# jemisjoky/ContracTN

Hardware: AMD Instinct MI355X
Metric: contractions/sec (MPS-100 overlap, bond=256, phys=4, fp32, stabilised split format) (higher is better)
Workload: dtype f32; 1 GPU; mps_overlap_100sites_D256_d4_zipper_R512; replicas_per_gpu=512, steps_per_contraction=199, bytes_min_per_contraction=205537284, parallelism=replicas x1

## Files before the change

contractn_amd/csrc/engine.hip:

```cpp
#include <hip/hip_runtime.h>

#include <cmath>
#include <cstdio>
#include <cstring>
#include <new>
#include <string>
#include <vector>

#include "plan.h"

#include "kernel_args.h"
#include "kernels_mfma.h"
#include "kernels_mfma_g.h"
#include "kernels_mfma_g64.h"
#include "kernels_mfma_h.h"
#include "kernels_mfma_ares.h"
#include "kernels_zip.h"
#include "kernels_zip64.h"
#include "kernels_zipl.h"
#include "kernels_sweep.h"
#include "kernels_mfma_lat.h"
#include "kernels_stream.h"

namespace ctn {

thread_local std::string g_err;

struct DevSwitches {
  int mfma_g = 1;
  int graph = 1;
  int mfma_bk = 0;
  int group = 1;
  int halve = 1;
  int lat_wg_per_cu_x2 = 2;
  int lat_max_t = 64;
  int splitk_fill_long = 2;
  int lat64_min_k = 512;
  int splitk = -1;
  int splitk_max = 0;
  int lat = -1;
  int hform = -1;
  int sweep = -1;
  int dot_tr = 1;
  int zip = -1;
  int zipl = -1;
  int zipl_max_r = 8;
  int g_big_min_k = 1024;
  int ares = -1;
  int ares_ntw = 0;
  int g_big = 1;
  int g_splitk = 1;
  int zipl_mp = 0;
  bool g_no_asm = false;
  const char* stamps = nullptr;
  int stamp_step = -1;
};
static DevSwitches read_dev_switches() {
  DevSwitches d;
  auto num = [](const char* name, int dflt) { const char* e = getenv(name); return e ? atoi(e) : dflt; };
  d.mfma_g = num("CTN_MFMA_G", 1);
  d.graph = num("CTN_GRAPH", 1);
  const int bk = num("CTN_MFMA_BK", 0);
  d.mfma_bk = (bk == 16 || bk == 32) ? bk : 0;
  d.splitk = num("CTN_SPLITK", -1);
  d.splitk_max = num("CTN_SPLITK_MAX", 0);
  d.lat = num("CTN_LAT", -1);
  d.hform = num("CTN_H", -1);
  d.zip = num("CTN_ZIP", -1);
  d.zipl = num("CTN_ZIPL", -1);
  d.zipl_max_r = num("CTN_ZIPL_MAX_R", 8);
  d.zipl_mp = num("CTN_ZIPL_MP", 0);
  d.g_splitk = num("CTN_G_SPLITK", 1);
  d.g_big = num("CTN_G_BIG", 1);
  d.ares = num("CTN_ARES", -1);
  d.ares_ntw = num("CTN_ARES_NTW", 0);
  d.g_big_min_k = num("CTN_G_BIG_MIN_K", 1024);
  d.dot_tr = num("CTN_DOT_TR", 1);
  d.sweep = num("CTN_SWEEP", -1);
  d.lat64_min_k = num("CTN_LAT64_MIN_K", 512);
  d.splitk_fill_long = num("CTN_SPLITK_FILL_LONG", 2);
  d.lat_max_t = num("CTN_LAT_MAX_T", 64);
  d.lat_wg_per_cu_x2 = num("CTN_LAT_WG_X2", 2);
  d.halve = num("CTN_HALVE_TILES", 1);
  d.group = num("CTN_GROUP", 1);
  d.g_no_asm = getenv("CTN_G_NO_ASM") != nullptr;
  d.stamps = getenv("CTN_DEBUG_STAMPS");
  d.stamp_step = num("CTN_DEBUG_STAMP_STEP", -1);
  return d;
}

#define HIPCHECK(expr)                                                                   \
  do {                                                                                   \
    hipError_t e_ = (expr);                                                              \
    if (e_ != hipSuccess) {                                                              \
      g_err = std::string(#expr) + ": " + hipGetErrorString(e_);                         \
      return CTN_HIP_ERROR;                                                              \
    }                                                                                    \
  } while (0)

struct DeviceGuard {
  int prev = -1;
  hipError_t err;
  explicit DeviceGuard(int dev) {
    if (hipGetDevice(&prev) != hipSuccess) { prev = -1; (void)hipGetLastError(); }
    err = prev == dev ? hipSuccess : hipSetDevice(dev);
    if (prev == dev) prev = -1;
  }
  ~DeviceGuard() { if (prev >= 0) (void)hipSetDevice(prev); }
};

struct Exec {
  const Plan* plan = nullptr;
  int device = 0;
  hipStream_t stream = nullptr;
  bool own_stream = false;
  int R = 1;
  int n_tensors = 0;
  int n_cu = 256;
  DevSwitches sw;
  int mfma_g = 1;
  int use_graph = 1;
  bool graph_warm = false;
  bool graph_aligned = true;
  hipGraphExec_t graph_exec = nullptr;
  struct ZipDesc { bool on = false; int64_t ldE = 0, ldXq = 0, ldXk = 0, ldYq = 0, ldYm = 0, ldC = 0; int Q = 0, U = 0, K1 = 0;
                   int zu = 128; };
  std::vector<ZipDesc> zip;
  std::vector<char> zip_skip;
  struct ZipLat { bool on = false, from_prev = false, feeds_next = false; int buf = 0, mp = 32; ZipDesc d; };
  std::vector<ZipLat> zl;
  std::vector<char> zl_skip;
  float* d_zl_slab[2] = {nullptr, nullptr};
  struct SweepDesc {
    bool on = false;
    std::vector<int> steps;
    int64_t ldIn = 0, ldOut = 0, ldWl = 0, ldWp = 0, ldX = 0;
    int J = 0, M = 0, D = 0, Pd = 0;
  };
  SweepDesc sweep;
  std::vector<char> sweep_role;
  int32_t* d_sweep_ids = nullptr;
  int64_t* d_sweep_off = nullptr;
  int32_t* d_sweep_slots = nullptr;
  double* d_sweep_a = nullptr;
  float* d_sweep_s = nullptr;
  double* d_sweep_z = nullptr;
  double* d_sweep_la = nullptr;
  double* d_sweep_ls = nullptr;
  std::vector<int> ares_ntw;
  struct DotTr { bool on = false; int Ka = 0, Kb = 0, x_is_a = 1; int64_t ldY = 0; };
  std::vector<DotTr> dot_tr;
  std::vector<int32_t> launched_tile;
  char* d_ws = nullptr;
  int32_t* d_tables = nullptr;
  int64_t* d_tables64 = nullptr;
  void** d_ptrs = nullptr;
  std::vector<void*> h_ptrs;
  bool ptrs_valid = false;
  double* d_partials = nullptr;
  double* d_scratch = nullptr;
  void* d_slab = nullptr;
  void* d_slab2 = nullptr;
  std::vector<int> step_partials;
  std::vector<int64_t> step_off;
  int64_t part_slots = 0;
  int64_t* d_stepOff = nullptr;
  int32_t* d_stepSlots = nullptr;
  double* d_log = nullptr;
// ... 617 lines not shown
      z.min_norm = P.min_norm;
      z.partC = E->d_partials + (size_t)E->step_off[s] * R;
      z.partC_stride = E->step_partials[s];
      const bool timed_z = E->timing_runs < E->timing_slots;
      const size_t ez = timed_z ? ((size_t)E->timing_runs * P.n_steps + s) * 2 : 0;
      if (timed_z) HIPCHECK(hipEventRecord(E->events[ez], E->stream));
      if ((int)E->launched_tile.size() != P.n_steps) E->launched_tile.assign(P.n_steps, 0);
      E->launched_tile[s] = (L.mp << 16) | ZM;
      const dim3 gz((unsigned)((int64_t)R * nub * S));
      z.dbg = nullptr;
      if (E->sw.stamps && (E->sw.stamp_step < 0 || E->sw.stamp_step == s)) {
        const size_t need = (size_t)gz.x;
        if (E->dbg_tiles < need) {
          if (E->d_dbg) (void)hipFree(E->d_dbg);
          HIPCHECK(hipMalloc((void**)&E->d_dbg, need * 64));
          E->dbg_tiles = need;
        }
        z.dbg = E->d_dbg;
        HIPCHECK(hipMemsetAsync(E->d_dbg, 0, E->dbg_tiles * 64, E->stream));
      }
      if (zd.Q == 4 && L.mp == 32) hipLaunchKernelGGL((k_zip_lat<4, 32>), gz, dim3(512), 0, E->stream, z);
      else if (zd.Q == 4) hipLaunchKernelGGL((k_zip_lat<4, 64>), gz, dim3(512), 0, E->stream, z);
      else hipLaunchKernelGGL((k_zip_lat<2, 64>), gz, dim3(512), 0, E->stream, z);
      if (!L.feeds_next || eager) {
        hipLaunchKernelGGL(k_zip_slab_sum, dim3((unsigned)E->step_partials[s], (unsigned)R), dim3(256), 0, E->stream,
                           (const float*)z.slabs_out, S, zd.U, (void* const*)E->d_ptrs, E->n_tensors, st.out, zd.ldC, z.partC,
                           z.partC_stride);
        if (eager && P.stabilize && s + 1 < P.n_steps) {
          const int64_t numel = P.tensors[st.out].numel;
          const dim3 g((unsigned)std::max<int64_t>(1, std::min<int64_t>((numel / 4 + 255) / 256, 2048)), R);
          hipLaunchKernelGGL(k_renorm<float>, g, dim3(256), 0, E->stream, (void* const*)E->d_ptrs, E->n_tensors, st.out, numel,
                             (const double*)z.partC, E->step_partials[s], E->step_partials[s], P.min_norm);
        }
      }
      if (timed_z) HIPCHECK(hipEventRecord(E->events[ez + 1], E->stream));
      continue;
    }
    if (!E->zip_skip.empty() && E->zip_skip[s]) {
      if ((int)E->launched_tile.size() != P.n_steps) E->launched_tile.assign(P.n_steps, 0);
      E->launched_tile[s] = (1 << 16) | 1;
      if (E->timing_runs < E->timing_slots) {
        const size_t e0 = ((size_t)E->timing_runs * P.n_steps + s) * 2;
        HIPCHECK(hipEventRecord(E->events[e0], E->stream));
        HIPCHECK(hipEventRecord(E->events[e0 + 1], E->stream));
      }
      continue;
    }
    if (!E->zip.empty() && E->zip[s].on) {
      const Exec::ZipDesc& zd = E->zip[s];
      const Step& s1 = P.steps[s - 1];
      ZipArgs z{};
      z.ptrs = E->d_ptrs; z.n_tensors = E->n_tensors;
      z.idE = s1.lhs; z.idX = s1.rhs; z.idY = st.rhs; z.idC = st.out;
      z.ldE = zd.ldE; z.ldXq = zd.ldXq; z.ldXk = zd.ldXk; z.ldYq = zd.ldYq; z.ldYm = zd.ldYm; z.ldC = zd.ldC;
      z.K1 = zd.K1; z.Q = zd.Q; z.U = zd.U;
      z.partE = nullptr; z.PE = 0; z.strideE = 0; z.numelE = 1.0;
      if (s1.lhs >= P.n_inputs && P.stabilize && !E->eager_rescale && P.steps[P.tensors[s1.lhs].producer].kernel != CTN_KERNEL_FUSED) {
        const int ps = P.tensors[s1.lhs].producer;
        z.partE = E->d_partials + (size_t)E->step_off[ps] * R;
        z.PE = z.strideE = E->step_partials[ps];
        z.numelE = (double)P.tensors[s1.lhs].numel;
      }
      z.min_norm = P.min_norm;
      z.partC = E->d_partials + (size_t)E->step_off[s] * R;
      z.partC_stride = E->step_partials[s];
      z.R = R; z.dbg = nullptr;
      const bool timed_z = E->timing_runs < E->timing_slots;
      const size_t ez = timed_z ? ((size_t)E->timing_runs * P.n_steps + s) * 2 : 0;
      if (timed_z) HIPCHECK(hipEventRecord(E->events[ez], E->stream));
      if ((int)E->launched_tile.size() != P.n_steps) E->launched_tile.assign(P.n_steps, 0);
      E->launched_tile[s] = (512 << 16) | (zd.zu == 64 ? 128 : 256);
      const int per = zd.U / zd.zu;
      if (E->sw.stamps && (E->sw.stamp_step < 0 || E->sw.stamp_step == s)) {
        const size_t need = (size_t)per * R;
        if (E->dbg_tiles < need) {
          if (E->d_dbg) (void)hipFree(E->d_dbg);
          HIPCHECK(hipMalloc((void**)&E->d_dbg, need * 64));
          E->dbg_tiles = need;
        }
        z.dbg = E->d_dbg;
        HIPCHECK(hipMemsetAsync(E->d_dbg, 0, E->dbg_tiles * 64, E->stream));
      }
      if (zd.zu == 64) hipLaunchKernelGGL(k_zip64_f32, dim3((unsigned)((int64_t)per * R)), dim3(512), 0, E->stream, z);
      else hipLaunchKernelGGL(k_zip_f32, dim3((unsigned)((int64_t)per * R)), dim3(512), 0, E->stream, z);
      if (E->eager_rescale && P.stabilize && s + 1 < P.n_steps) {
        const int64_t numel = P.tensors[st.out].numel;
        const dim3 g((unsigned)std::max<int64_t>(1, std::min<int64_t>((numel / 4 + 255) / 256, 2048)), R);
        hipLaunchKernelGGL(k_renorm<float>, g, dim3(256), 0, E->stream, (void* const*)E->d_ptrs, E->n_tensors, st.out, numel,
                           (const double*)z.partC, E->step_partials[s], E->step_partials[s], P.min_norm);
      }
      if (timed_z) HIPCHECK(hipEventRecord(E->events[ez + 1], E->stream));
      continue;
    }
    if (st.kernel == CTN_KERNEL_FUSED) {
      if (E->timing_runs < E->timing_slots) {
        const size_t e0 = ((size_t)E->timing_runs * P.n_steps + s) * 2;
        HIPCHECK(hipEventRecord(E->events[e0], E->stream));
        HIPCHECK(hipEventRecord(E->events[e0 + 1], E->stream));
      }
      continue;
    }
    StepArgs a;
    const int32_t* T = E->d_tables;
    const int64_t* T8 = E->d_tables64;
    a.obA = T8 + st.t.obA; a.obB = T8 + st.t.obB; a.obC = T8 + st.t.obC;
    a.omA = T + st.t.omA; a.omC = T + st.t.omC;
    a.onB = T + st.t.onB; a.onC = T + st.t.onC;
    a.okA = T + st.t.okA; a.okB = T + st.t.okB;
    a.ptrs = E->d_ptrs;
    auto part_of = [&](int id, const double** p, int32_t* cnt, int32_t* stride, double* numel) {
      *p = nullptr; *cnt = 0; *stride = 0; *numel = 1;
      if (id >= P.n_inputs && P.stabilize && !E->eager_rescale && P.steps[P.tensors[id].producer].kernel != CTN_KERNEL_FUSED) {
        const int ps = P.tensors[id].producer;
        *p = E->d_partials + (size_t)E->step_off[ps] * R;
        *cnt = *stride = E->step_partials[ps];
        *numel = (double)P.tensors[id].numel;
      }
    };
    part_of(st.lhs, &a.partA, &a.PA, &a.strideA, &a.numelA);
    part_of(st.rhs, &a.partB, &a.PB, &a.strideB, &a.numelB);
    part_of(st.lhs2, &a.partA2, &a.PA2, &a.strideA2, &a.numelA2);
    a.obA2 = T8 + st.t.obA2; a.omA2 = T + st.t.omA2; a.okA2 = T + st.t.okA2;
    a.idA2 = st.lhs2 >= 0 ? st.lhs2 : E->n_tensors - 1;
    a.krX = st.krX; a.krY = st.krY;
    a.epw = st.epw | (st.epw_split ? 0x100 : 0);
    double* part_dst = E->d_partials + (size_t)E->step_off[s] * R;
    const int part_stride = E->step_partials[s];
    a.partC = st.collapse ? E->d_scratch : part_dst;
    a.partC_stride = st.collapse ? st.blocks : part_stride;
    int collapse_blocks = st.blocks;
    bool reduced = false;
    bool do_collapse = st.collapse;
    a.min_norm = P.min_norm;
    a.Bt = (int32_t)st.Bt; a.M = (int32_t)st.M; a.N = (int32_t)st.N; a.K = (int32_t)st.K;
    a.idA = st.lhs; a.idB = st.rhs >= 0 ? st.rhs : E->n_tensors - 1; a.idC = st.out;
    a.n_tensors = E->n_tensors;
    const int row_tile = (st.kernel == CTN_KERNEL_MFMA_F32 && st.tileM == 64) ? 64 : kTileM;
    a.tiles_m = (int32_t)((st.M + row_tile - 1) / row_tile);
    a.tiles_n = (int32_t)((st.N + kTileN - 1) / kTileN);
    a.blocks_per_replica = st.blocks;
    a.R = R;
    a.c_vec = (st.cvec && (s + 1 < P.n_steps || E->outs_aligned16)) ? 1 : 0;
    a.dbg = nullptr;
    a.ks_slab = nullptr; a.ks_numelC = 0; a.ks_S = 0; a.ks_chunk = 0;
    a.ohA = T8 + st.t.ohA; a.ohB = T8 + st.t.ohB; a.ohC = T8 + st.t.ohC;
    a.olA = T + st.t.olA; a.olB = T + st.t.olB; a.olC = T + st.t.olC;
    a.H = (int32_t)st.H; a.L = (int32_t)st.L; a.Nv = (int32_t)st.Nv;
    a.sAn = (int32_t)st.sAn; a.sBn = (int32_t)st.sBn;
    a.dNq = make_fastdiv((st.Nv + st.vecw - 1) / st.vecw);
    a.dL = make_fastdiv(st.L);
    a.dNv = make_fastdiv(st.Nv);

    const bool timed = E->timing_runs < E->timing_slots;
    const size_t ev0 = timed ? ((size_t)E->timing_runs * P.n_steps + s) * 2 : 0;
    if (timed) HIPCHECK(hipEventRecord(E->events[ev0], E->stream));
    if ((int)E->launched_tile.size() != P.n_steps) E->launched_tile.assign(P.n_steps, 0);
    auto used_tile = [&](int tm, int tn) { E->launched_tile[s] = (tm << 16) | tn; };
    switch (st.kernel) {
      case CTN_KERNEL_MFMA_F32: {
        const int64_t total = (int64_t)st.blocks * R;
        if (total >= (1LL << 31)) { g_err = "grid too large"; return CTN_UNSUPPORTED; }
        if (const int ntw_av = (int)E->ares_ntw.size() == P.n_steps ? E->ares_ntw[s] : 0) {
          const int ntw = ntw_av & 0xffff, avec = ntw_av >> 16;
          const int wgs = (int)(st.Bt * (st.N / AR_TN / ntw));
          a.partC = E->d_scratch; a.partC_stride = wgs;
          do_collapse = true; collapse_blocks = wgs;
          used_tile(256, std::min(AR_TN * ntw, 32768));
// ... 1197 lines not shown
```

contractn_amd/csrc/kernels_zip.h:

```cpp
#pragma once
#include "kernels_mfma_g.h"

namespace ctn {

struct ZipArgs {
  void* const* ptrs;
  int32_t n_tensors, idE, idX, idY, idC;
  int64_t ldE;
  int64_t ldXq, ldXk;
  int64_t ldYq, ldYm;
  int64_t ldC;
  int32_t K1, Q, U;
  const double* partE;
  int32_t PE, strideE;
  double numelE, min_norm;
  double* partC;
  int32_t partC_stride, R;
  unsigned long long* dbg;
};

constexpr int ZM = 256, ZU = 128, ZK = 16, ZSTG = 8192;
constexpr int ZST = 3;

__global__ __launch_bounds__(512, 1) void k_zip_f32(ZipArgs a) {
  __shared__ __attribute__((aligned(16))) float smem[ZST * ZSTG + 16];
  double* red = reinterpret_cast<double*>(smem + ZST * ZSTG);

  const int tid = threadIdx.x;
  const int lane = tid & 63;
  const int w = __builtin_amdgcn_readfirstlane(tid >> 6);
  const int kh = w >> 2, ub = w & 3;
  const int l31 = lane & 31, h = lane >> 5;
  const int nwg = gridDim.x, bid = blockIdx.x;
  const int xcd = bid & 7, slot = bid >> 3, q8 = nwg >> 3, r8 = nwg & 7;
  const int pid = (xcd < r8 ? xcd * (q8 + 1) : r8 * (q8 + 1) + (xcd - r8) * q8) + slot;
  const int per = a.U / ZU;
  const int r = pid / per;
  const int t_ = pid - r * per;
  const int u0 = t_ * ZU;
#ifdef CTN_STAMPS
  if (a.dbg && tid == 0) a.dbg[(size_t)pid * 8 + 0] = __builtin_amdgcn_s_memtime();
#endif
  void* const* tp = a.ptrs + (size_t)r * a.n_tensors;
  const float* __restrict__ E = (const float*)tp[a.idE];
  const float* __restrict__ X = (const float*)tp[a.idX] + u0;
  const float* __restrict__ Y = (const float*)tp[a.idY];
  float* __restrict__ C = (float*)tp[a.idC];

  const int T1 = a.K1 / ZK;
  constexpr int T2 = (ZM / 2) / ZK;
  const int TQ = T1 + T2, TT = a.Q * TQ;

  const float* const rE0 = E + (int64_t)(4 * ub) * a.ldE;
  const float* rE = rE0;
  const float* rX = X + (int64_t)(4 * ub) * a.ldXk;
  const float* rY = Y + (int64_t)(4 * ub) * a.ldYm;
  const int offE = 4 * lane, offX = h * (int)a.ldXk + 4 * l31;
  const int64_t stepE = (int64_t)ZK * a.ldE, stepX = (int64_t)ZK * a.ldXk, stepY = (int64_t)ZK * a.ldYm;
  const int64_t nextX = a.ldXq - (int64_t)a.K1 * a.ldXk, nextY = a.ldYq - (int64_t)(ZM / 2) * a.ldYm;
  const int64_t halfY = (int64_t)(ZM / 2) * a.ldYm;
  int rq_s = 0, rq_left = TT;
  auto request_issue = [&](int stage) {
    float* st = smem + stage * ZSTG;
    if (rq_s < T1) {
#pragma unroll
      for (int i = 0; i < 4; ++i) glds16(rE + i * a.ldE + offE, st + (4 * ub + i) * ZM);
#pragma unroll
      for (int i = 0; i < 2; ++i) glds16(rX + 2 * i * a.ldXk + offX, st + 4096 + (4 * ub + 2 * i) * ZU);
    } else {
#pragma unroll
      for (int hf = 0; hf < 2; ++hf)
#pragma unroll
        for (int i = 0; i < 4; ++i) glds16(rY + hf * halfY + i * a.ldYm + offE, st + hf * 4096 + (4 * ub + i) * ZM);
    }
  };
  auto request_step = [&]() {
    const bool p1 = rq_s < T1;
    --rq_left;
    ++rq_s;
    const bool wrap = rq_s == TQ;
    rq_s = wrap ? 0 : rq_s;
    rE = wrap ? rE0 : rE + (p1 ? stepE : 0);
    rX += (p1 ? stepX : 0) + (wrap ? nextX : 0);
    rY += (p1 ? 0 : stepY) + (wrap ? nextY : 0);
  };

  f32x16 acc1[4], acc2[8];
#pragma unroll
  for (int i = 0; i < 4; ++i)
#pragma unroll
    for (int e = 0; e < 16; ++e) acc1[i][e] = 0.f;
#pragma unroll
  for (int i = 0; i < 8; ++i)
#pragma unroll
    for (int e = 0; e < 16; ++e) acc2[i][e] = 0.f;

#pragma unroll
  for (int i = 0; i < ZST - 1; ++i) {
    if (kh == 0) request_issue(i);
    request_step();
  }
  double pve = 0.0;
  if (a.partE) {
    const double* __restrict__ pr = a.partE + (size_t)r * a.strideE;
    pve = pr[min(lane, a.PE - 1)];
    if (a.PE > 64)
      for (int i = lane + 64; i < a.PE; i += 64) pve += pr[i];
  }
  __builtin_amdgcn_sched_barrier(0);
  __builtin_amdgcn_s_waitcnt(0x0F70);
  __builtin_amdgcn_s_barrier();
#ifdef CTN_STAMPS
  if (a.dbg && tid == 0) a.dbg[(size_t)pid * 8 + 1] = __builtin_amdgcn_s_memtime();
#endif

  constexpr int bar_at = 3;
  int st_cur = 0, st_nxt = 1, st_req = ZST - 1, t = 0;
#ifdef CTN_STAMPS
  unsigned long long wait_vm = 0, wait_bar = 0;
#endif
  auto middle = [&]() {
    __builtin_amdgcn_sched_barrier(0);
#ifdef CTN_STAMPS
    const unsigned long long s0 = __builtin_amdgcn_s_memtime();
#endif
    __builtin_amdgcn_s_waitcnt(0x0F70);
#ifdef CTN_STAMPS
    const unsigned long long s1 = __builtin_amdgcn_s_memtime();
#endif
    __builtin_amdgcn_s_barrier();
#ifdef CTN_STAMPS
    const unsigned long long s2 = __builtin_amdgcn_s_memtime();
    wait_vm += s1 - s0;
    wait_bar += s2 - s1;
#endif
    if (kh == 0 && rq_left > 0) request_issue(st_req);
    __builtin_amdgcn_sched_barrier(0);
  };
  auto advance = [&]() {
    st_req = st_cur;
    st_cur = st_nxt;
    st_nxt = st_nxt == ZST - 1 ? 0 : st_nxt + 1;
    ++t;
  };
  float fa[2][4], fb[2], fy[2][8];

  for (int q = 0; q < a.Q; ++q) {
    for (int s = 0; s < T1; ++s) {
      const float* cA = smem + st_cur * ZSTG + h * ZM + kh * (ZM / 2) + l31;
      const float* cB = smem + st_cur * ZSTG + 4096 + h * ZU + ub * 32 + l31;
#pragma unroll
      for (int i = 0; i < 4; ++i) fa[0][i] = cA[32 * i];
      fb[0] = cB[0];
#pragma unroll
      for (int kk = 0; kk < ZK / 2; ++kk) {
        const int c = kk & 1, nx = c ^ 1;
        if (kk + 1 < ZK / 2) {
#pragma unroll
          for (int i = 0; i < 4; ++i) fa[nx][i] = cA[2 * (kk + 1) * ZM + 32 * i];
          fb[nx] = cB[2 * (kk + 1) * ZU];
        }
        if (kk == bar_at + 1) request_step();
#pragma unroll
        for (int i = 0; i < 4; ++i)
          acc1[i] = __builtin_amdgcn_mfma_f32_32x32x2f32(fa[c][i], fb[c], acc1[i], 0, 0, 0);
        __builtin_amdgcn_sched_group_barrier(0x008, 1, 0);
        __builtin_amdgcn_sched_group_barrier(0x100, 5, 0);
#pragma unroll
        for (int i = 0; i < 3; ++i) {
          __builtin_amdgcn_sched_group_barrier(0x004, 12, 0);
          __builtin_amdgcn_sched_group_barrier(0x008, 1, 0);
        }
        if (kk == bar_at) middle();
      }
      advance();
    }
#pragma unroll
    for (int ms = 0; ms < T2; ++ms) {
      const float* cY = smem + st_cur * ZSTG + kh * 4096 + (4 * h) * ZM + l31;
#pragma unroll
      for (int nb = 0; nb < 8; ++nb) fy[0][nb] = cY[32 * nb];
#pragma unroll
      for (int kk = 0; kk < 8; ++kk) {
        const int c = kk & 1, nx = c ^ 1;
        if (kk + 1 < 8) {
#pragma unroll
          for (int nb = 0; nb < 8; ++nb) fy[nx][nb] = cY[(8 * ((kk + 1) / 4) + (kk + 1) % 4) * ZM + 32 * nb];
        }
        const float tq = acc1[ms / 2][4 * (2 * (ms & 1) + kk / 4) + kk % 4];
        if (kk == bar_at + 1) request_step();
#pragma unroll
        for (int nb = 0; nb < 8; ++nb)
          acc2[nb] = __builtin_amdgcn_mfma_f32_32x32x2f32(fy[c][nb], tq, acc2[nb], 0, 0, 0);
        __builtin_amdgcn_sched_group_barrier(0x008, 1, 0);
        __builtin_amdgcn_sched_group_barrier(0x100, 8, 0);
#pragma unroll
        for (int i = 0; i < 7; ++i) {
          __builtin_amdgcn_sched_group_barrier(0x004, 6, 0);
          __builtin_amdgcn_sched_group_barrier(0x008, 1, 0);
        }
        if (kk == bar_at) middle();
      }
      advance();
    }
#pragma unroll
    for (int i = 0; i < 4; ++i)
#pragma unroll
      for (int e = 0; e < 16; ++e) acc1[i][e] = 0.f;
  }
#ifdef CTN_STAMPS
  if (a.dbg && tid == 0) {
    a.dbg[(size_t)pid * 8 + 2] = __builtin_amdgcn_s_memtime();
    a.dbg[(size_t)pid * 8 + 5] = wait_vm;
    a.dbg[(size_t)pid * 8 + 6] = wait_bar;
  }
  if (a.dbg && tid == 448) a.dbg[(size_t)pid * 8 + 7] = wait_vm + wait_bar;
#endif

  f32x16 mine[4], give[4];
  if (kh == 0) {
#pragma unroll
    for (int i = 0; i < 4; ++i) { mine[i] = acc2[i]; give[i] = acc2[4 + i]; }
  } else {
#pragma unroll
    for (int i = 0; i < 4; ++i) { mine[i] = acc2[4 + i]; give[i] = acc2[i]; }
  }
#pragma unroll
  for (int round = 0; round < 2; ++round) {
    __builtin_amdgcn_s_waitcnt(0xC07F);
    __builtin_amdgcn_s_barrier();
    float4* xo = reinterpret_cast<float4*>(smem + w * 2048) + lane;
#pragma unroll
    for (int i = 0; i < 2; ++i)
#pragma unroll
      for (int qd = 0; qd < 4; ++qd)
        xo[(i * 4 + qd) * 64] = make_float4(give[2 * round + i][4 * qd], give[2 * round + i][4 * qd + 1],
                                            give[2 * round + i][4 * qd + 2], give[2 * round + i][4 * qd + 3]);
    __builtin_amdgcn_s_waitcnt(0xC07F);
    __builtin_amdgcn_s_barrier();
    const float4* xi = reinterpret_cast<const float4*>(smem + (w ^ 4) * 2048) + lane;
#pragma unroll
    for (int i = 0; i < 2; ++i)
#pragma unroll
      for (int qd = 0; qd < 4; ++qd) {
        const float4 o = xi[(i * 4 + qd) * 64];
        const float ov[4] = {o.x, o.y, o.z, o.w};
#pragma unroll
        for (int e = 0; e < 4; ++e) {
          const float m = mine[2 * round + i][4 * qd + e];
          mine[2 * round + i][4 * qd + e] = kh == 0 ? m + ov[e] : ov[e] + m;
        }
      }
  }
#ifdef CTN_STAMPS
  if (a.dbg && tid == 0) a.dbg[(size_t)pid * 8 + 4] = __builtin_amdgcn_s_memtime();
#endif

  pve = lane < a.PE ? pve : 0.0;
#pragma unroll
  for (int o = 32; o > 0; o >>= 1) pve += __shfl_xor(pve, o, 64);
  const float nE = (float)pve;
  const float scE = (a.partE && nE > (float)a.min_norm) ? nE / (float)a.numelE : 1.f;
  const float iE = 1.0f / scE;
  float asum = 0.f;
  float* __restrict__ row = C + (int64_t)(u0 + 32 * ub + l31) * a.ldC + 4 * h;
#pragma unroll
  for (int i = 0; i < 4; ++i) {
    const int nb = 4 * kh + i;
#pragma unroll
    for (int g = 0; g < 4; ++g) {
      float4 v;
      v.x = mine[i][4 * g + 0] * iE; v.y = mine[i][4 * g + 1] * iE; v.z = mine[i][4 * g + 2] * iE; v.w = mine[i][4 * g + 3] * iE;
      *reinterpret_cast<float4*>(row + 32 * nb + 8 * g) = v;
      asum += (fabsf(v.x) + fabsf(v.y)) + (fabsf(v.z) + fabsf(v.w));
    }
  }
  double part = (double)asum;
#pragma unroll
  for (int o = 32; o > 0; o >>= 1) part += __shfl_xor(part, o, 64);
  if (lane == 0) red[w] = part;
  __builtin_amdgcn_s_waitcnt(0xC07F);
  __builtin_amdgcn_s_barrier();
  if (tid == 0) {
    double tot = 0.0;
#pragma unroll
    for (int i = 0; i < 8; ++i) tot += red[i];
    a.partC[(size_t)r * a.partC_stride + t_] = tot;
  }
#ifdef CTN_STAMPS
  if (a.dbg && tid == 0) a.dbg[(size_t)pid * 8 + 3] = __builtin_amdgcn_s_memtime();
#endif
}

}
```

Before: 5166 contractions/s.

## Hand-schedule zip kernel inner loops with inline asm MFMA/LDS interleave

Adds an inline-assembly path for the zip kernel's two phases, explicitly interleaving ds_read prefetches of the next k-slice with v_mfma_f32_32x32x2 instructions and using b128 LDS reads in phase 2. A permlane32_swap epilogue remaps the accumulator layout to match what the later reduction expects. The aim is to hide LDS latency behind MFMA issue, which the compiler scheduler was not doing well. The asm path is the default, and the C++ path stays available through an environment switch. The hand-coded register layout and hazard nops are fragile and could break correctness or create stalls.

```diff
diff --git a/contractn_amd/csrc/engine.hip b/contractn_amd/csrc/engine.hip
--- a/contractn_amd/csrc/engine.hip
+++ b/contractn_amd/csrc/engine.hip
@@ -52,6 +52,7 @@
   int g_splitk = 1;
   int zipl_mp = 0;
   bool g_no_asm = false;
+  bool zip_no_asm = false;
   const char* stamps = nullptr;
   int stamp_step = -1;
 };
@@ -84,6 +85,7 @@
   d.halve = num("CTN_HALVE_TILES", 1);
   d.group = num("CTN_GROUP", 1);
   d.g_no_asm = getenv("CTN_G_NO_ASM") != nullptr;
+  d.zip_no_asm = getenv("CTN_ZIP_NO_ASM") != nullptr;
   d.stamps = getenv("CTN_DEBUG_STAMPS");
   d.stamp_step = num("CTN_DEBUG_STAMP_STEP", -1);
   return d;
@@ -867,7 +869,8 @@
         HIPCHECK(hipMemsetAsync(E->d_dbg, 0, E->dbg_tiles * 64, E->stream));
       }
       if (zd.zu == 64) hipLaunchKernelGGL(k_zip64_f32, dim3((unsigned)((int64_t)per * R)), dim3(512), 0, E->stream, z);
-      else hipLaunchKernelGGL(k_zip_f32, dim3((unsigned)((int64_t)per * R)), dim3(512), 0, E->stream, z);
+      else if (E->sw.zip_no_asm) hipLaunchKernelGGL(k_zip_f32<false>, dim3((unsigned)((int64_t)per * R)), dim3(512), 0, E->stream, z);
+      else hipLaunchKernelGGL(k_zip_f32<true>, dim3((unsigned)((int64_t)per * R)), dim3(512), 0, E->stream, z);
       if (E->eager_rescale && P.stabilize && s + 1 < P.n_steps) {
         const int64_t numel = P.tensors[st.out].numel;
         const dim3 g((unsigned)std::max<int64_t>(1, std::min<int64_t>((numel / 4 + 255) / 256, 2048)), R);
diff --git a/contractn_amd/csrc/kernels_zip.h b/contractn_amd/csrc/kernels_zip.h
--- a/contractn_amd/csrc/kernels_zip.h
+++ b/contractn_amd/csrc/kernels_zip.h
@@ -1,5 +1,6 @@
 #pragma once
 #include "kernels_mfma_g.h"
+#include "kernels_zip_asm.inc"
 
 namespace ctn {
 
@@ -22,6 +23,7 @@
 constexpr int ZM = 256, ZU = 128, ZK = 16, ZSTG = 8192;
 constexpr int ZST = 3;
 
+template <bool ASM>
 __global__ __launch_bounds__(512, 1) void k_zip_f32(ZipArgs a) {
   __shared__ __attribute__((aligned(16))) float smem[ZST * ZSTG + 16];
   double* red = reinterpret_cast<double*>(smem + ZST * ZSTG);
@@ -115,7 +117,7 @@
 #endif
 
   constexpr int bar_at = 3;
-  int st_cur = 0, st_nxt = 1, st_req = ZST - 1, t = 0;
+  int st_cur = 0, st_nxt = 1, st_req = ZST - 1;
 #ifdef CTN_STAMPS
   unsigned long long wait_vm = 0, wait_bar = 0;
 #endif
@@ -141,10 +143,61 @@
     st_req = st_cur;
     st_cur = st_nxt;
     st_nxt = st_nxt == ZST - 1 ? 0 : st_nxt + 1;
-    ++t;
   };
   float fa[2][4], fb[2], fy[2][8];
 
+  if constexpr (ASM) {
+    const unsigned vA0 = lds_addr(smem + h * ZM + kh * (ZM / 2) + l31);
+    const unsigned vB0 = lds_addr(smem + 4096 + h * ZU + ub * 32 + l31);
+    const unsigned vY0 = lds_addr(smem + kh * 4096 + (4 * h) * ZM + 4 * l31);
+    zip_f32x4 y[2][2];
+    for (int q = 0; q < a.Q; ++q) {
+      for (int s = 0; s < T1; ++s) {
+        const unsigned vA = vA0 + st_cur * (ZSTG * 4), vB = vB0 + st_cur * (ZSTG * 4);
+        __builtin_amdgcn_sched_barrier(0);
+        zip_p1_load0(acc1, fa, fb, vA, vB);
+        if (s == 0) zip_p1_step<0, true>(acc1, fa, fb, vA, vB);
+        else zip_p1_step<0>(acc1, fa, fb, vA, vB);
+        zip_p1_step<1>(acc1, fa, fb, vA, vB);
+        zip_p1_step<2>(acc1, fa, fb, vA, vB);
+        zip_p1_step<3>(acc1, fa, fb, vA, vB);
+        middle();
+        zip_p1_step<4>(acc1, fa, fb, vA, vB);
+        __builtin_amdgcn_sched_barrier(0);
+        request_step();
+        __builtin_amdgcn_sched_barrier(0);
+        zip_p1_step<5>(acc1, fa, fb, vA, vB);
+        zip_p1_step<6>(acc1, fa, fb, vA, vB);
+        zip_p1_step<7>(acc1, fa, fb, vA, vB);
+        __builtin_amdgcn_sched_barrier(0);
+        advance();
+      }
+#pragma unroll
+      for (int ms = 0; ms < T2; ++ms) {
+        const unsigned vY = vY0 + st_cur * (ZSTG * 4);
+        const f32x16& tq = acc1[ms / 2];
+        const int gq = 8 * (ms & 1);
+        __builtin_amdgcn_sched_barrier(0);
+        if (ms == 0) asm volatile("s_nop 7\n\ts_nop 7\n\ts_nop 3" ::: "memory");
+        zip_p2_load0(y[0], vY);
+        zip_p2_step<0>(acc2, y[0], y[1], tq[gq + 0], vY);
+        zip_p2_step<1>(acc2, y[1], y[0], tq[gq + 1], vY);
+        zip_p2_step<2>(acc2, y[0], y[1], tq[gq + 2], vY);
+        zip_p2_step<3>(acc2, y[1], y[0], tq[gq + 3], vY);
+        middle();
+        zip_p2_step<4>(acc2, y[0], y[1], tq[gq + 4], vY);
+        __builtin_amdgcn_sched_barrier(0);
+        request_step();
+        __builtin_amdgcn_sched_barrier(0);
+        zip_p2_step<5>(acc2, y[1], y[0], tq[gq + 5], vY);
+        zip_p2_step<6>(acc2, y[0], y[1], tq[gq + 6], vY);
+        zip_p2_step<7>(acc2, y[1], y[0], tq[gq + 7], vY);
+        __builtin_amdgcn_sched_barrier(0);
+        advance();
+      }
+    }
+    asm volatile("s_nop 7\n\ts_nop 7\n\ts_nop 3" ::: "memory");
+  } else
   for (int q = 0; q < a.Q; ++q) {
     for (int s = 0; s < T1; ++s) {
       const float* cA = smem + st_cur * ZSTG + h * ZM + kh * (ZM / 2) + l31;
@@ -252,6 +305,24 @@
         }
       }
   }
+  if constexpr (ASM) {
+    f32x16 o[4];
+#pragma unroll
+    for (int i = 0; i < 4; ++i)
+#pragma unroll
+      for (int e = 0; e < 4; ++e) {
+        const auto r0 = __builtin_amdgcn_permlane32_swap(__float_as_uint(mine[e][4 * i]), __float_as_uint(mine[e][4 * i + 1]),
+                                                         false, false);
+        const auto r1 = __builtin_amdgcn_permlane32_swap(__float_as_uint(mine[e][4 * i + 2]),
+                                                         __float_as_uint(mine[e][4 * i + 3]), false, false);
+        o[i][e] = __uint_as_float(r0[0]);
+        o[i][8 + e] = __uint_as_float(r0[1]);
+        o[i][4 + e] = __uint_as_float(r1[0]);
+        o[i][12 + e] = __uint_as_float(r1[1]);
+      }
+#pragma unroll
+    for (int i = 0; i < 4; ++i) mine[i] = o[i];
+  }
 #ifdef CTN_STAMPS
   if (a.dbg && tid == 0) a.dbg[(size_t)pid * 8 + 4] = __builtin_amdgcn_s_memtime();
 #endif
diff --git a/contractn_amd/csrc/kernels_zip_asm.inc b/contractn_amd/csrc/kernels_zip_asm.inc
--- /dev/null
+++ b/contractn_amd/csrc/kernels_zip_asm.inc
@@ -0,0 +1,282 @@
+#pragma once
+
+namespace ctn {
+
+typedef float zip_f32x4 __attribute__((ext_vector_type(4)));
+
+#define CTN_ZIP_P1_LOAD0 \
+  "ds_read_b32 %[fa00], %[vA] offset:0\n\t" \
+  "ds_read_b32 %[fa01], %[vA] offset:128\n\t" \
+  "ds_read_b32 %[fa02], %[vA] offset:256\n\t" \
+  "ds_read_b32 %[fa03], %[vA] offset:384\n\t" \
+  "ds_read_b32 %[fb0], %[vB] offset:0\n\t" \
+  "s_waitcnt lgkmcnt(0)\n\t"
+#define CTN_ZIP_P1_STEP_0Z \
+  "v_mfma_f32_32x32x2_f32 %[a0], %[fa00], %[fb0], 0\n\t" \
+  "ds_read_b32 %[fa10], %[vA] offset:2048\n\t" \
+  "ds_read_b32 %[fa11], %[vA] offset:2176\n\t" \
+  "ds_read_b32 %[fa12], %[vA] offset:2304\n\t" \
+  "ds_read_b32 %[fa13], %[vA] offset:2432\n\t" \
+  "ds_read_b32 %[fb1], %[vB] offset:1024\n\t" \
+  "v_mfma_f32_32x32x2_f32 %[a1], %[fa01], %[fb0], 0\n\t" \
+  "v_mfma_f32_32x32x2_f32 %[a2], %[fa02], %[fb0], 0\n\t" \
+  "v_mfma_f32_32x32x2_f32 %[a3], %[fa03], %[fb0], 0\n\t" \
+  "s_waitcnt lgkmcnt(0)\n\t"
+#define CTN_ZIP_P1_STEP_0 \
+  "v_mfma_f32_32x32x2_f32 %[a0], %[fa00], %[fb0], %[a0]\n\t" \
+  "ds_read_b32 %[fa10], %[vA] offset:2048\n\t" \
+  "ds_read_b32 %[fa11], %[vA] offset:2176\n\t" \
+  "ds_read_b32 %[fa12], %[vA] offset:2304\n\t" \
+  "ds_read_b32 %[fa13], %[vA] offset:2432\n\t" \
+  "ds_read_b32 %[fb1], %[vB] offset:1024\n\t" \
+  "v_mfma_f32_32x32x2_f32 %[a1], %[fa01], %[fb0], %[a1]\n\t" \
+  "v_mfma_f32_32x32x2_f32 %[a2], %[fa02], %[fb0], %[a2]\n\t" \
+  "v_mfma_f32_32x32x2_f32 %[a3], %[fa03], %[fb0], %[a3]\n\t" \
+  "s_waitcnt lgkmcnt(0)\n\t"
+#define CTN_ZIP_P1_STEP_1 \
+  "v_mfma_f32_32x32x2_f32 %[a0], %[fa10], %[fb1], %[a0]\n\t" \
+  "ds_read_b32 %[fa00], %[vA] offset:4096\n\t" \
+  "ds_read_b32 %[fa01], %[vA] offset:4224\n\t" \
+  "ds_read_b32 %[fa02], %[vA] offset:4352\n\t" \
+  "ds_read_b32 %[fa03], %[vA] offset:4480\n\t" \
+  "ds_read_b32 %[fb0], %[vB] offset:2048\n\t" \
+  "v_mfma_f32_32x32x2_f32 %[a1], %[fa11], %[fb1], %[a1]\n\t" \
+  "v_mfma_f32_32x32x2_f32 %[a2], %[fa12], %[fb1], %[a2]\n\t" \
+  "v_mfma_f32_32x32x2_f32 %[a3], %[fa13], %[fb1], %[a3]\n\t" \
+  "s_waitcnt lgkmcnt(0)\n\t"
+#define CTN_ZIP_P1_STEP_2 \
+  "v_mfma_f32_32x32x2_f32 %[a0], %[fa00], %[fb0], %[a0]\n\t" \
+  "ds_read_b32 %[fa10], %[vA] offset:6144\n\t" \
+  "ds_read_b32 %[fa11], %[vA] offset:6272\n\t" \
+  "ds_read_b32 %[fa12], %[vA] offset:6400\n\t" \
+  "ds_read_b32 %[fa13], %[vA] offset:6528\n\t" \
+  "ds_read_b32 %[fb1], %[vB] offset:3072\n\t" \
+  "v_mfma_f32_32x32x2_f32 %[a1], %[fa01], %[fb0], %[a1]\n\t" \
+  "v_mfma_f32_32x32x2_f32 %[a2], %[fa02], %[fb0], %[a2]\n\t" \
+  "v_mfma_f32_32x32x2_f32 %[a3], %[fa03], %[fb0], %[a3]\n\t" \
+  "s_waitcnt lgkmcnt(0)\n\t"
+#define CTN_ZIP_P1_STEP_3 \
+  "v_mfma_f32_32x32x2_f32 %[a0], %[fa10], %[fb1], %[a0]\n\t" \
+  "ds_read_b32 %[fa00], %[vA] offset:8192\n\t" \
+  "ds_read_b32 %[fa01], %[vA] offset:8320\n\t" \
+  "ds_read_b32 %[fa02], %[vA] offset:8448\n\t" \
+  "ds_read_b32 %[fa03], %[vA] offset:8576\n\t" \
+  "ds_read_b32 %[fb0], %[vB] offset:4096\n\t" \
+  "v_mfma_f32_32x32x2_f32 %[a1], %[fa11], %[fb1], %[a1]\n\t" \
+  "v_mfma_f32_32x32x2_f32 %[a2], %[fa12], %[fb1], %[a2]\n\t" \
+  "v_mfma_f32_32x32x2_f32 %[a3], %[fa13], %[fb1], %[a3]\n\t" \
+  "s_waitcnt lgkmcnt(0)\n\t"
+#define CTN_ZIP_P1_STEP_4 \
+  "v_mfma_f32_32x32x2_f32 %[a0], %[fa00], %[fb0], %[a0]\n\t" \
+  "ds_read_b32 %[fa10], %[vA] offset:10240\n\t" \
+  "ds_read_b32 %[fa11], %[vA] offset:10368\n\t" \
+  "ds_read_b32 %[fa12], %[vA] offset:10496\n\t" \
+  "ds_read_b32 %[fa13], %[vA] offset:10624\n\t" \
+  "ds_read_b32 %[fb1], %[vB] offset:5120\n\t" \
+  "v_mfma_f32_32x32x2_f32 %[a1], %[fa01], %[fb0], %[a1]\n\t" \
+  "v_mfma_f32_32x32x2_f32 %[a2], %[fa02], %[fb0], %[a2]\n\t" \
+  "v_mfma_f32_32x32x2_f32 %[a3], %[fa03], %[fb0], %[a3]\n\t" \
+  "s_waitcnt lgkmcnt(0)\n\t"
+#define CTN_ZIP_P1_STEP_5 \
+  "v_mfma_f32_32x32x2_f32 %[a0], %[fa10], %[fb1], %[a0]\n\t" \
+  "ds_read_b32 %[fa00], %[vA] offset:12288\n\t" \
+  "ds_read_b32 %[fa01], %[vA] offset:12416\n\t" \
+  "ds_read_b32 %[fa02], %[vA] offset:12544\n\t" \
+  "ds_read_b32 %[fa03], %[vA] offset:12672\n\t" \
+  "ds_read_b32 %[fb0], %[vB] offset:6144\n\t" \
+  "v_mfma_f32_32x32x2_f32 %[a1], %[fa11], %[fb1], %[a1]\n\t" \
+  "v_mfma_f32_32x32x2_f32 %[a2], %[fa12], %[fb1], %[a2]\n\t" \
+  "v_mfma_f32_32x32x2_f32 %[a3], %[fa13], %[fb1], %[a3]\n\t" \
+  "s_waitcnt lgkmcnt(0)\n\t"
+#define CTN_ZIP_P1_STEP_6 \
+  "v_mfma_f32_32x32x2_f32 %[a0], %[fa00], %[fb0], %[a0]\n\t" \
+  "ds_read_b32 %[fa10], %[vA] offset:14336\n\t" \
+  "ds_read_b32 %[fa11], %[vA] offset:14464\n\t" \
+  "ds_read_b32 %[fa12], %[vA] offset:14592\n\t" \
+  "ds_read_b32 %[fa13], %[vA] offset:14720\n\t" \
+  "ds_read_b32 %[fb1], %[vB] offset:7168\n\t" \
+  "v_mfma_f32_32x32x2_f32 %[a1], %[fa01], %[fb0], %[a1]\n\t" \
+  "v_mfma_f32_32x32x2_f32 %[a2], %[fa02], %[fb0], %[a2]\n\t" \
+  "v_mfma_f32_32x32x2_f32 %[a3], %[fa03], %[fb0], %[a3]\n\t" \
+  "s_waitcnt lgkmcnt(0)\n\t"
+#define CTN_ZIP_P1_STEP_7 \
+  "v_mfma_f32_32x32x2_f32 %[a0], %[fa10], %[fb1], %[a0]\n\t" \
+  "v_mfma_f32_32x32x2_f32 %[a1], %[fa11], %[fb1], %[a1]\n\t" \
+  "v_mfma_f32_32x32x2_f32 %[a2], %[fa12], %[fb1], %[a2]\n\t" \
+  "v_mfma_f32_32x32x2_f32 %[a3], %[fa13], %[fb1], %[a3]\n\t"
+#define CTN_ZIP_P2_LOAD0 \
+  "ds_read_b128 %[yn0], %[vY] offset:0\n\t" \
+  "ds_read_b128 %[yn1], %[vY] offset:512\n\t" \
+  "s_waitcnt lgkmcnt(0)\n\t"
+#define CTN_ZIP_P2_STEP_0 \
+  "v_mfma_f32_32x32x2_f32 %[c0], %[y0], %[t], %[c0]\n\t" \
+  "ds_read_b128 %[yn0], %[vY] offset:1024\n\t" \
+  "ds_read_b128 %[yn1], %[vY] offset:1536\n\t" \
+  "v_mfma_f32_32x32x2_f32 %[c1], %[y1], %[t], %[c1]\n\t" \
+  "v_mfma_f32_32x32x2_f32 %[c2], %[y2], %[t], %[c2]\n\t" \
+  "v_mfma_f32_32x32x2_f32 %[c3], %[y3], %[t], %[c3]\n\t" \
+  "v_mfma_f32_32x32x2_f32 %[c4], %[y4], %[t], %[c4]\n\t" \
+  "v_mfma_f32_32x32x2_f32 %[c5], %[y5], %[t], %[c5]\n\t" \
+  "v_mfma_f32_32x32x2_f32 %[c6], %[y6], %[t], %[c6]\n\t" \
+  "v_mfma_f32_32x32x2_f32 %[c7], %[y7], %[t], %[c7]\n\t" \
+  "s_waitcnt lgkmcnt(0)\n\t"
+#define CTN_ZIP_P2_STEP_1 \
+  "v_mfma_f32_32x32x2_f32 %[c0], %[y0], %[t], %[c0]\n\t" \
+  "ds_read_b128 %[yn0], %[vY] offset:2048\n\t" \
+  "ds_read_b128 %[yn1], %[vY] offset:2560\n\t" \
+  "v_mfma_f32_32x32x2_f32 %[c1], %[y1], %[t], %[c1]\n\t" \
+  "v_mfma_f32_32x32x2_f32 %[c2], %[y2], %[t], %[c2]\n\t" \
+  "v_mfma_f32_32x32x2_f32 %[c3], %[y3], %[t], %[c3]\n\t" \
+  "v_mfma_f32_32x32x2_f32 %[c4], %[y4], %[t], %[c4]\n\t" \
+  "v_mfma_f32_32x32x2_f32 %[c5], %[y5], %[t], %[c5]\n\t" \
+  "v_mfma_f32_32x32x2_f32 %[c6], %[y6], %[t], %[c6]\n\t" \
+  "v_mfma_f32_32x32x2_f32 %[c7], %[y7], %[t], %[c7]\n\t" \
+  "s_waitcnt lgkmcnt(0)\n\t"
+#define CTN_ZIP_P2_STEP_2 \
+  "v_mfma_f32_32x32x2_f32 %[c0], %[y0], %[t], %[c0]\n\t" \
+  "ds_read_b128 %[yn0], %[vY] offset:3072\n\t" \
+  "ds_read_b128 %[yn1], %[vY] offset:3584\n\t" \
+  "v_mfma_f32_32x32x2_f32 %[c1], %[y1], %[t], %[c1]\n\t" \
+  "v_mfma_f32_32x32x2_f32 %[c2], %[y2], %[t], %[c2]\n\t" \
+  "v_mfma_f32_32x32x2_f32 %[c3], %[y3], %[t], %[c3]\n\t" \
+  "v_mfma_f32_32x32x2_f32 %[c4], %[y4], %[t], %[c4]\n\t" \
+  "v_mfma_f32_32x32x2_f32 %[c5], %[y5], %[t], %[c5]\n\t" \
+  "v_mfma_f32_32x32x2_f32 %[c6], %[y6], %[t], %[c6]\n\t" \
+  "v_mfma_f32_32x32x2_f32 %[c7], %[y7], %[t], %[c7]\n\t" \
+  "s_waitcnt lgkmcnt(0)\n\t"
+#define CTN_ZIP_P2_STEP_3 \
+  "v_mfma_f32_32x32x2_f32 %[c0], %[y0], %[t], %[c0]\n\t" \
+  "ds_read_b128 %[yn0], %[vY] offset:8192\n\t" \
+  "ds_read_b128 %[yn1], %[vY] offset:8704\n\t" \
+  "v_mfma_f32_32x32x2_f32 %[c1], %[y1], %[t], %[c1]\n\t" \
+  "v_mfma_f32_32x32x2_f32 %[c2], %[y2], %[t], %[c2]\n\t" \
+  "v_mfma_f32_32x32x2_f32 %[c3], %[y3], %[t], %[c3]\n\t" \
+  "v_mfma_f32_32x32x2_f32 %[c4], %[y4], %[t], %[c4]\n\t" \
+  "v_mfma_f32_32x32x2_f32 %[c5], %[y5], %[t], %[c5]\n\t" \
+  "v_mfma_f32_32x32x2_f32 %[c6], %[y6], %[t], %[c6]\n\t" \
+  "v_mfma_f32_32x32x2_f32 %[c7], %[y7], %[t], %[c7]\n\t" \
+  "s_waitcnt lgkmcnt(0)\n\t"
+#define CTN_ZIP_P2_STEP_4 \
+  "v_mfma_f32_32x32x2_f32 %[c0], %[y0], %[t], %[c0]\n\t" \
+  "ds_read_b128 %[yn0], %[vY] offset:9216\n\t" \
+  "ds_read_b128 %[yn1], %[vY] offset:9728\n\t" \
+  "v_mfma_f32_32x32x2_f32 %[c1], %[y1], %[t], %[c1]\n\t" \
+  "v_mfma_f32_32x32x2_f32 %[c2], %[y2], %[t], %[c2]\n\t" \
+  "v_mfma_f32_32x32x2_f32 %[c3], %[y3], %[t], %[c3]\n\t" \
+  "v_mfma_f32_32x32x2_f32 %[c4], %[y4], %[t], %[c4]\n\t" \
+  "v_mfma_f32_32x32x2_f32 %[c5], %[y5], %[t], %[c5]\n\t" \
+  "v_mfma_f32_32x32x2_f32 %[c6], %[y6], %[t], %[c6]\n\t" \
+  "v_mfma_f32_32x32x2_f32 %[c7], %[y7], %[t], %[c7]\n\t" \
+  "s_waitcnt lgkmcnt(0)\n\t"
+#define CTN_ZIP_P2_STEP_5 \
+  "v_mfma_f32_32x32x2_f32 %[c0], %[y0], %[t], %[c0]\n\t" \
+  "ds_read_b128 %[yn0], %[vY] offset:10240\n\t" \
+  "ds_read_b128 %[yn1], %[vY] offset:10752\n\t" \
+  "v_mfma_f32_32x32x2_f32 %[c1], %[y1], %[t], %[c1]\n\t" \
+  "v_mfma_f32_32x32x2_f32 %[c2], %[y2], %[t], %[c2]\n\t" \
+  "v_mfma_f32_32x32x2_f32 %[c3], %[y3], %[t], %[c3]\n\t" \
+  "v_mfma_f32_32x32x2_f32 %[c4], %[y4], %[t], %[c4]\n\t" \
+  "v_mfma_f32_32x32x2_f32 %[c5], %[y5], %[t], %[c5]\n\t" \
+  "v_mfma_f32_32x32x2_f32 %[c6], %[y6], %[t], %[c6]\n\t" \
+  "v_mfma_f32_32x32x2_f32 %[c7], %[y7], %[t], %[c7]\n\t" \
+  "s_waitcnt lgkmcnt(0)\n\t"
+#define CTN_ZIP_P2_STEP_6 \
+  "v_mfma_f32_32x32x2_f32 %[c0], %[y0], %[t], %[c0]\n\t" \
+  "ds_read_b128 %[yn0], %[vY] offset:11264\n\t" \
+  "ds_read_b128 %[yn1], %[vY] offset:11776\n\t" \
+  "v_mfma_f32_32x32x2_f32 %[c1], %[y1], %[t], %[c1]\n\t" \
+  "v_mfma_f32_32x32x2_f32 %[c2], %[y2], %[t], %[c2]\n\t" \
+  "v_mfma_f32_32x32x2_f32 %[c3], %[y3], %[t], %[c3]\n\t" \
+  "v_mfma_f32_32x32x2_f32 %[c4], %[y4], %[t], %[c4]\n\t" \
+  "v_mfma_f32_32x32x2_f32 %[c5], %[y5], %[t], %[c5]\n\t" \
+  "v_mfma_f32_32x32x2_f32 %[c6], %[y6], %[t], %[c6]\n\t" \
+  "v_mfma_f32_32x32x2_f32 %[c7], %[y7], %[t], %[c7]\n\t" \
+  "s_waitcnt lgkmcnt(0)\n\t"
+#define CTN_ZIP_P2_STEP_7 \
+  "v_mfma_f32_32x32x2_f32 %[c0], %[y0], %[t], %[c0]\n\t" \
+  "v_mfma_f32_32x32x2_f32 %[c1], %[y1], %[t], %[c1]\n\t" \
+  "v_mfma_f32_32x32x2_f32 %[c2], %[y2], %[t], %[c2]\n\t" \
+  "v_mfma_f32_32x32x2_f32 %[c3], %[y3], %[t], %[c3]\n\t" \
+  "v_mfma_f32_32x32x2_f32 %[c4], %[y4], %[t], %[c4]\n\t" \
+  "v_mfma_f32_32x32x2_f32 %[c5], %[y5], %[t], %[c5]\n\t" \
+  "v_mfma_f32_32x32x2_f32 %[c6], %[y6], %[t], %[c6]\n\t" \
+  "v_mfma_f32_32x32x2_f32 %[c7], %[y7], %[t], %[c7]\n\t"
+
+#define CTN_ZIP_P1_OPERANDS                                                                              \
+  [a0] "+v"(acc[0]), [a1] "+v"(acc[1]), [a2] "+v"(acc[2]), [a3] "+v"(acc[3]),                            \
+  [fa00] "+v"(fa[0][0]), [fa01] "+v"(fa[0][1]), [fa02] "+v"(fa[0][2]), [fa03] "+v"(fa[0][3]),            \
+  [fa10] "+v"(fa[1][0]), [fa11] "+v"(fa[1][1]), [fa12] "+v"(fa[1][2]), [fa13] "+v"(fa[1][3]),            \
+  [fb0] "+v"(fb[0]), [fb1] "+v"(fb[1])
+#define CTN_ZIP_P2_INPUTS                                                                                \
+  [y0] "v"(y[0][0]), [y1] "v"(y[0][1]), [y2] "v"(y[0][2]), [y3] "v"(y[0][3]),                            \
+  [y4] "v"(y[1][0]), [y5] "v"(y[1][1]), [y6] "v"(y[1][2]), [y7] "v"(y[1][3]), [t] "v"(t), [vY] "v"(vY)
+#define CTN_ZIP_P2_ACC                                                                                   \
+  [c0] "+v"(acc[0]), [c1] "+v"(acc[1]), [c2] "+v"(acc[2]), [c3] "+v"(acc[3]),                            \
+  [c4] "+v"(acc[4]), [c5] "+v"(acc[5]), [c6] "+v"(acc[6]), [c7] "+v"(acc[7])
+
+template <int KK, bool Z = false>
+__device__ __forceinline__ void zip_p1_step(f32x16 (&acc)[4], float (&fa)[2][4], float (&fb)[2], unsigned vA,
+                                            unsigned vB) {
+  if constexpr (Z) {
+    static_assert(KK == 0, "the zero-C form is the first k-step");
+    asm volatile(CTN_ZIP_P1_STEP_0Z : CTN_ZIP_P1_OPERANDS : [vA] "v"(vA), [vB] "v"(vB) : "memory");
+  } else if constexpr (KK == 0) {
+    asm volatile(CTN_ZIP_P1_STEP_0 : CTN_ZIP_P1_OPERANDS : [vA] "v"(vA), [vB] "v"(vB) : "memory");
+  } else if constexpr (KK == 1) {
+    asm volatile(CTN_ZIP_P1_STEP_1 : CTN_ZIP_P1_OPERANDS : [vA] "v"(vA), [vB] "v"(vB) : "memory");
+  } else if constexpr (KK == 2) {
+    asm volatile(CTN_ZIP_P1_STEP_2 : CTN_ZIP_P1_OPERANDS : [vA] "v"(vA), [vB] "v"(vB) : "memory");
+  } else if constexpr (KK == 3) {
+    asm volatile(CTN_ZIP_P1_STEP_3 : CTN_ZIP_P1_OPERANDS : [vA] "v"(vA), [vB] "v"(vB) : "memory");
+  } else if constexpr (KK == 4) {
+    asm volatile(CTN_ZIP_P1_STEP_4 : CTN_ZIP_P1_OPERANDS : [vA] "v"(vA), [vB] "v"(vB) : "memory");
+  } else if constexpr (KK == 5) {
+    asm volatile(CTN_ZIP_P1_STEP_5 : CTN_ZIP_P1_OPERANDS : [vA] "v"(vA), [vB] "v"(vB) : "memory");
+  } else if constexpr (KK == 6) {
+    asm volatile(CTN_ZIP_P1_STEP_6 : CTN_ZIP_P1_OPERANDS : [vA] "v"(vA), [vB] "v"(vB) : "memory");
+  } else if constexpr (KK == 7) {
+    asm volatile(CTN_ZIP_P1_STEP_7 : CTN_ZIP_P1_OPERANDS : [vA] "v"(vA), [vB] "v"(vB) : "memory");
+  }
+}
+__device__ __forceinline__ void zip_p1_load0(f32x16 (&acc)[4], float (&fa)[2][4], float (&fb)[2], unsigned vA,
+                                             unsigned vB) {
+  asm volatile(CTN_ZIP_P1_LOAD0 : CTN_ZIP_P1_OPERANDS : [vA] "v"(vA), [vB] "v"(vB) : "memory");
+}
+
+template <int KK>
+__device__ __forceinline__ void zip_p2_step(f32x16 (&acc)[8], const zip_f32x4 (&y)[2], zip_f32x4 (&yn)[2], float t,
+                                            unsigned vY) {
+  if constexpr (KK == 0) {
+    asm volatile(CTN_ZIP_P2_STEP_0 : CTN_ZIP_P2_ACC, [yn0] "+v"(yn[0]), [yn1] "+v"(yn[1])
+                 : CTN_ZIP_P2_INPUTS : "memory");
+  } else if constexpr (KK == 1) {
+    asm volatile(CTN_ZIP_P2_STEP_1 : CTN_ZIP_P2_ACC, [yn0] "+v"(yn[0]), [yn1] "+v"(yn[1])
+                 : CTN_ZIP_P2_INPUTS : "memory");
+  } else if constexpr (KK == 2) {
+    asm volatile(CTN_ZIP_P2_STEP_2 : CTN_ZIP_P2_ACC, [yn0] "+v"(yn[0]), [yn1] "+v"(yn[1])
+                 : CTN_ZIP_P2_INPUTS : "memory");
+  } else if constexpr (KK == 3) {
+    asm volatile(CTN_ZIP_P2_STEP_3 : CTN_ZIP_P2_ACC, [yn0] "+v"(yn[0]), [yn1] "+v"(yn[1])
+                 : CTN_ZIP_P2_INPUTS : "memory");
+  } else if constexpr (KK == 4) {
+    asm volatile(CTN_ZIP_P2_STEP_4 : CTN_ZIP_P2_ACC, [yn0] "+v"(yn[0]), [yn1] "+v"(yn[1])
+                 : CTN_ZIP_P2_INPUTS : "memory");
+  } else if constexpr (KK == 5) {
+    asm volatile(CTN_ZIP_P2_STEP_5 : CTN_ZIP_P2_ACC, [yn0] "+v"(yn[0]), [yn1] "+v"(yn[1])
+                 : CTN_ZIP_P2_INPUTS : "memory");
+  } else if constexpr (KK == 6) {
+    asm volatile(CTN_ZIP_P2_STEP_6 : CTN_ZIP_P2_ACC, [yn0] "+v"(yn[0]), [yn1] "+v"(yn[1])
+                 : CTN_ZIP_P2_INPUTS : "memory");
+  } else if constexpr (KK == 7) {
+    asm volatile(CTN_ZIP_P2_STEP_7 : CTN_ZIP_P2_ACC : CTN_ZIP_P2_INPUTS : "memory");
+  }
+}
+__device__ __forceinline__ void zip_p2_load0(zip_f32x4 (&yn)[2], unsigned vY) {
+  asm volatile(CTN_ZIP_P2_LOAD0 : [yn0] "+v"(yn[0]), [yn1] "+v"(yn[1]) : [vY] "v"(vY) : "memory");
+}
+
+#undef CTN_ZIP_P1_OPERANDS
+#undef CTN_ZIP_P2_INPUTS
+#undef CTN_ZIP_P2_ACC
+
+}
```

Measured after the change: 5210 contractions/s (median of 6 runs). Within noise of the previous version (+0.9%).
